# jayHuggie/PathTracer_CUDA_Interactive

Measured on AMD Instinct MI355X. Metric: Msamples/sec (rays x spp x bounces = intersect() calls per second), scenes/cbox/cbox.xml 640x480 spp=64, higher is better.
Workload: dtype f32

## Files before the change

pathtracer_cuda_interactive_amd/csrc/pt_api.hip:

```cpp
#include <cmath>
#include <cstdio>
#include <cstdlib>
#include <cstring>
#include <initializer_list>
#include <iterator>
#include <limits>
#include <mutex>
#include <type_traits>

#include "pt_scene.h"
#include "pt_transform.h"
#include "pt_denoise.h"
#include "pt_gradient.h"
#include "pt_temporal.h"
#include "pt_kernels.h"
#include "pt_kernel_q.h"
#include "pt_query.h"

using namespace ptk;

static thread_local std::string g_err;
int pt_fail(int code, const std::string& msg) { g_err = msg; return code; }
static int fail(int code, const std::string& msg) { return pt_fail(code, msg); }

// ... 249 lines not shown
    if (c.sched.inner >= 1000 && c.which != 1) return {};
    static_assert(std::size(kV2Schedules) == 9, "the index list below enumerates kV2Schedules");
    int si = -1;
    for (int k = 0; k < (int)std::size(kV2Schedules); k++)
        if (kV2Schedules[k].thresh == c.sched.thresh && kV2Schedules[k].inner == c.sched.inner && kV2Schedules[k].minw == c.sched.minw) si = k;
    return among<0, 1, 2, 3, 4, 5, 6, 7, 8>(si, [&](auto SI) { return among<0, 1, 2, 3>(c.res, [&](auto R) {
           return among<false, true>(c.nee, [&](auto N) { return among<false, true>(c.list, [&](auto LI) {
           static constexpr V2Schedule s = kV2Schedules[PT_CONST(SI)];
           if constexpr (!v2_compiled(PT_CONST(R), false, s, 0, PT_CONST(N), PT_CONST(LI))) return TraceEntry{};
           else return among<0, 1, 2>(c.spec, [&](auto SP) { return among<false, true>(c.prune, [&](auto P) {
           return among<false, true>(c.stats, [&](auto S) {
               if constexpr (v2_compiled(PT_CONST(R), PT_CONST(P), s, PT_CONST(SP), PT_CONST(N), PT_CONST(LI)))
                   return v2k<PT_CONST(R), PT_CONST(P), PT_CONST(S), s.thresh, s.inner, s.minw, PT_CONST(SP), PT_CONST(N), PT_CONST(LI)>();
               else return TraceEntry{}; }); }); }); }); }); }); });
}
#undef PT_CONST

void launch_trace(const pt_scene* S, const TraceChoice& c, const TraceEntry& e, int grid, hipStream_t stream, const RenderDev& rd,
                  const LdsPlan& lp, const QParams& qp, float4* samples) {
    void* const fn = const_cast<void*>(e.fn);
    if (c.family == 3)
        hipLaunchKernelGGL(reinterpret_cast<TraceFnQ>(fn), dim3(grid), dim3(c.block_threads), lp.total, stream, S->dev, rd, lp, qp,
                           samples, S->work_counter(), S->counters());
    else if (c.sweep)
        hipLaunchKernelGGL(reinterpret_cast<SweepFn>(fn), dim3(grid), dim3(c.block_threads), lp.total, stream, S->dev, rd, lp,
                           samples, S->work_counter(), S->counters(), SweepLayoutDev{S->sweep_tab.p, S->sweep.count, 0u});
    else
        hipLaunchKernelGGL(reinterpret_cast<TraceFn>(fn), dim3(grid), dim3(c.block_threads), lp.total, stream, S->dev, rd, lp,
                           samples, S->work_counter(), S->counters());
}

int read_slot_sums(const pt_scene* S, unsigned long long* out) {
    std::vector<unsigned long long> raw(kTimelineBase);
    HIP_TRY(hipMemcpy(raw.data(), S->counters(), raw.size() * sizeof(unsigned long long), hipMemcpyDeviceToHost));
    std::fill(out, out + kSlotStride, 0ull);
    for (int s = 0; s < kCounterSlots; s++)
        for (int k = 0; k < kSlotStride; k++) out[k] += raw[(size_t)s * kSlotStride + k];
    return PT_OK;
}

int launch_grid(int num_cus, int blocks_per_cu, uint64_t work_items, int block_threads = kBlock) {
    const uint64_t blocks_needed = (work_items + (uint64_t)block_threads - 1) / (uint64_t)block_threads;
    return (int)std::max<uint64_t>(1, std::min<uint64_t>((uint64_t)num_cus * (uint64_t)blocks_per_cu, blocks_needed));
}

struct RowSel {
    int begin, step, count;
};

int select_rows(const pt_render_params* p, RowSel* out) {
// ... 1190 lines not shown
    else if (k == "top_cache") S->opt_top_cache = value;
    else if (k == "fast_tree") S->opt_fast_tree = value;
    else if (k == "lds_budget_kb") S->opt_lds_budget_kb = value;
    else if (k == "chunk") S->opt_chunk = value;
    else if (k == "item_order") S->opt_item_order = value;
    else if (k == "specialize") S->opt_specialize = value;
    else if (k == "timing_frames") {
        if (value < 0 || value > 4096) return fail(PT_ERR_INVALID_ARG, "timing_frames must be 0 .. 4096");
        S->opt_timing_frames = value;
    }
    else if (k == "kernel") { if (value < 1 || value > 3) return fail(PT_ERR_INVALID_ARG, "kernel must be 1, 2 or 3"); S->opt_kernel = value; }
    else if (k == "frames_in_flight") {
        if (value < 1 || value > kMaxFramesInFlight) return fail(PT_ERR_INVALID_ARG, "frames_in_flight must be 1 .. " + std::to_string(kMaxFramesInFlight));
        S->opt_frames_in_flight = value;
    }
    else if (k == "q_target") S->opt_q_target = value;
    else if (k == "q_swap") S->opt_q_swap = value;
    else if (k == "q_low") S->opt_q_low = value;
    else if (k == "v2_thresh") S->opt_v2_thresh = value;
    else if (k == "v2_inner") S->opt_v2_inner = value;
    else if (k == "v2_minw") S->opt_v2_minw = value;
    else if (k == "reg_stack") { if (value != 0 && value != 1) return fail(PT_ERR_INVALID_ARG, "reg_stack must be 0 or 1"); S->opt_reg_stack = value; }
    else if (k == "leaf_sweep") { if (value != 0 && value != 1) return fail(PT_ERR_INVALID_ARG, "leaf_sweep must be 0 or 1"); S->opt_leaf_sweep = value; }
    else if (k == "query_refill") { if (value < 0 || value > 64) return fail(PT_ERR_INVALID_ARG, "query_refill must be 0 (automatic) .. 64"); S->opt_query_refill = value; }
    else if (k == "query_guides") { if (value < 0 || value > 2) return fail(PT_ERR_INVALID_ARG, "query_guides must be 0 (automatic), 1 or 2"); S->opt_query_guides = value; }
    else if (k == "query_blocks") { if (value < 0 || value > 4096) return fail(PT_ERR_INVALID_ARG, "query_blocks must be 0 (automatic) .. 4096"); S->opt_query_blocks = value; }
    else if (k == "tree_cost") { if (value != 0 && value != 1) return fail(PT_ERR_INVALID_ARG, "tree_cost must be 0 or 1"); S->opt_tree_cost = value; }
    else if (k == "rebuild_at_permille") {
        if (value != 0 && value < 1001) return fail(PT_ERR_INVALID_ARG, "rebuild_at_permille must be 0 (never) or at least 1001");
        S->opt_rebuild_at = value;
    }
    else return fail(PT_ERR_INVALID_ARG, "unknown option " + k);
    return PT_OK;
}

int pt_scene_get_info(pt_scene* S, const char* key, int64_t* value) {
    if (!S || !key || !value) return fail(PT_ERR_INVALID_ARG, "null argument");
    const std::string k(key);
    TraceChoice next;
    (void)choose_trace(S, k == "vgprs_pruned" ? PT_TRAVERSAL_PRUNED : PT_TRAVERSAL_EXACT, false, false, &next);
    DeviceGuard guard;
    unsigned long long c[kSlotStride];
    if (k == "grid") *value = S->info_grid;
    else if (k == "lds_bytes") *value = S->info_lds_bytes;
    else if (k == "lds_scene") *value = S->info_lds_scene;
    else if (k == "residency") *value = next.res;
// ... 29 lines not shown
    else if (k == "transforms") *value = S->transforms;
    else if (k == "rebuilds") *value = S->rebuilds;
    else if (k == "rebuilds_auto") *value = S->rebuilds_auto;
    else if (k == "rebuild_adopted") *value = S->rebuild_adopted;
    else if (k == "rebuild_cost_permille") *value = S->rebuild_cost_permille;
    else if (k == "tree_cost0_bits" || k == "tree_cost1_bits") {
        const int t = k[9] - '0';
        const double c = (S->cost_on() && (t == 0 || S->have_fast)) ? S->cost_now[t] : 0.0;
        *value = c > 0.0 ? __builtin_bit_cast(int64_t, c) : 0;
    }
    else if (k == "tree_cost0_permille" || k == "tree_cost1_permille") {
        const int t = k[9] - '0';
        *value = (S->cost_on() && (t == 0 || S->have_fast)) ? cost_permille(S, t) : 1000;
    }
    else if (k == "refit_shape0" || k == "refit_shape1") {
        const ptf::Plan& pl = S->refit_plan[k[11] - '0'];
        *value = !pl.built ? 0 : pl.whole_tree ? 1 : pl.narrow_top < pl.levels - 1 ? 2 : 3;
    }
    else if (k == "kernel") *value = S->info_kernel;
    else if (k == "trace_variant") *value = S->info_trace_variant;
    else if (k == "path_bank") *value = S->info_path_bank;
    else if (k == "leaf_sweep") *value = S->info_leaf_sweep;
    else if (k == "sweep_boxes") *value = S->sweep_groups;
    else if (k == "reg_stack") *value = S->info_reg_stack;
    else if (k == "block_threads") *value = S->info_kernel == 3 ? kQBlock : kBlock;
    else if (k == "frames_in_flight") *value = S->opt_frames_in_flight;
    else if (k == "query_chunk") *value = ptq::kQueryChunk;
    else if (k == "query_guides") *value = S->info_query_guides;
    else if (k == "query_grid") *value = S->info_query_grid;
    else if (k.rfind("qdiag", 0) == 0 && k.size() >= 6 && k.size() <= 7 && k.find_first_not_of("0123456789", 5) == std::string::npos &&
             std::stoi(k.substr(5)) < 11) {
        int rc = synced_slot_sums(S, guard, c);
        if (rc) return rc;
        *value = (int64_t)c[4 + std::stoi(k.substr(5))];
    }
    else if (k.rfind("diag", 0) == 0 && k.size() >= 5 && k.size() <= 7 && k.find_first_not_of("0123456789", 4) == std::string::npos &&
             std::stoi(k.substr(4)) < 8 + kNumCounters - kTimelineBase) {
        unsigned long long v = 0;
        const int idx = std::stoi(k.substr(4));
        if (idx < 8) {
            int rc = synced_slot_sums(S, guard, c);
            if (rc) return rc;
            v = c[4 + idx];
        } else {
            if (int grc = guard.enter(S->device)) return grc;
            HIP_TRY(hipStreamSynchronize(S->last_stream));
// ... 113 lines not shown
```

pathtracer_cuda_interactive_amd/csrc/pt_kernels.h:

```cpp
#pragma once

#include <hip/hip_runtime.h>

#include <type_traits>

#include "pt_layout.h"
#include "pt_leaf_sweep.h"
#include "pt_math.h"
#include "pt_path_bank.h"
#include "pt_path_index.h"
#include "pt_sweep_layout.h"
#include "pt_temporal.h"
#include "pt_trace.h"

namespace ptk {

using namespace ptl;


#ifndef PT_BLOCK
#define PT_BLOCK 256
#endif
constexpr int kBlock = PT_BLOCK;
constexpr uint32_t kMaxChunk = 256;

__device__ __forceinline__ uint32_t lane_rank(unsigned long long mask) {
    return __builtin_amdgcn_mbcnt_hi((uint32_t)(mask >> 32), __builtin_amdgcn_mbcnt_lo((uint32_t)mask, 0u));
}

__device__ __forceinline__ unsigned long long wave_sum(unsigned long long v) {
    for (int off = 32; off > 0; off >>= 1) v += __shfl_down(v, off, 64);
    return v;
}

// ... 247 lines not shown
    constexpr bool REG = false;
#include "pt_trace_v2_body.h"
}

template <int RES, bool PRUNE, bool STATS, int MINW>
__global__ __launch_bounds__(kBlock, (kBlock > 256 ? 1 : MINW)) void trace_kernel_v2_reg(SceneDev scn, RenderDev rp, LdsPlan lp,
                                                              float4* __restrict__ samples,
                                                              uint32_t* __restrict__ work_counter,
                                                              unsigned long long* __restrict__ counters) {
    constexpr int THRESH = 40, INNER = 162, SPEC = 2;
    constexpr bool NEE = false, LIST = false, REG = true;
#include "pt_trace_v2_body.h"
}

#ifndef PT_SWEEP_LEAF_STEPS
#define PT_SWEEP_LEAF_STEPS 4
#endif
#ifndef PT_SWEEP_THRESH
#define PT_SWEEP_THRESH 48
#endif
struct SweepLayoutDev {
    const unsigned char* tab;
    uint32_t groups;
    uint32_t pad;
};
struct SweepKernelArgs {
    SceneDev scn; RenderDev rp; LdsPlan lp; float4* samples; uint32_t* work_counter; unsigned long long* counters; SweepLayoutDev sweep;
};
static_assert(offsetof(SweepKernelArgs, rp) == offsetof(TraceKernelArgs, rp), "reload_render_args reads rp at TraceKernelArgs' offset");

__device__ __forceinline__ ptd::SceneView make_sweep_view(const SceneDev& scn, const LdsPlan& lp, const SweepLayoutDev& sweep,
                                                          unsigned char* smem) {
    const uint32_t slots_off = sweep_slots_off(sweep.groups);
    stage_to_lds(smem + lp.nodes_off, sweep.tab, slots_off);
    const DPrim* gslots = reinterpret_cast<const DPrim*>(sweep.tab + slots_off);
    DPrim* lslots = reinterpret_cast<DPrim*>(smem + lp.nodes_off + slots_off);
    for (uint32_t i = threadIdx.x; i < (uint32_t)scn.num_prims; i += blockDim.x) {
        const float4 a = ptd::ld4(gslots + i, 0), b = ptd::ld4(gslots + i, 1), c = ptd::ld4(gslots + i, 2);
        DPrim g;
        g.v[0] = a.x; g.v[1] = a.y; g.v[2] = a.z; g.v[3] = a.w; g.v[4] = b.x; g.v[5] = b.y; g.v[6] = b.z; g.v[7] = b.w; g.v[8] = c.x;
        g.info = __builtin_bit_cast(int32_t, c.y); g.light = __builtin_bit_cast(int32_t, c.z); g.pad = __builtin_bit_cast(int32_t, c.w);
        const DPrim r = sweep_stage_record(g);
        float4* d = reinterpret_cast<float4*>(lslots + i);
        d[0] = make_float4(r.v[0], r.v[1], r.v[2], r.v[3]);
        d[1] = make_float4(r.v[4], r.v[5], r.v[6], r.v[7]);
        d[2] = make_float4(r.v[8], c.y, c.z, c.w);
    }
    stage_to_lds(smem + lp.prims_off, scn.prims, (uint32_t)scn.num_prims * sizeof(DPrim));
    stage_to_lds(smem + lp.normals_off, scn.normals, (uint32_t)scn.num_prims * sizeof(DNormals));
    stage_to_lds(smem + lp.mats_off, scn.materials, (uint32_t)scn.num_materials * sizeof(DMaterial));
    stage_to_lds(smem + lp.emis_off, scn.emission, (uint32_t)scn.num_emission * sizeof(DEmission));
    __syncthreads();
    ptd::SceneView sv;
    sv.top_nodes = nullptr;
    sv.top_count = 0;
    sv.nodes = reinterpret_cast<const DNode*>(smem + lp.nodes_off);
    sv.prims = reinterpret_cast<const DPrim*>(smem + lp.prims_off);
    sv.normals = reinterpret_cast<const DNormals*>(smem + lp.normals_off);
    sv.materials = reinterpret_cast<const DMaterial*>(smem + lp.mats_off);
    sv.emission = reinterpret_cast<const DEmission*>(smem + lp.emis_off);
    sv.node_stride = kLdsNodeStride;
    sv.oct_stride = sweep_box_pitch(sweep.groups);
    sv.lights = scn.lights;
    sv.num_emission = scn.num_emission;
    sv.root_ref = scn.root_ref;
    sv.fixed_order = scn.fixed_order;
    sv.ref_nodes = scn.ref_nodes; sv.ref_path = scn.ref_path; sv.ref_anc = scn.ref_anc; sv.ref_levels = scn.ref_levels;
    sv.bg = ptm::mk(scn.bg[0], scn.bg[1], scn.bg[2]);
    return sv;
}

template <int MINW>
__global__ __launch_bounds__(kBlock, (kBlock > 256 ? 1 : MINW)) void trace_kernel_v2_sweep(SceneDev scn, RenderDev rp, LdsPlan lp,
                                                                float4* __restrict__ samples,
                                                                uint32_t* __restrict__ work_counter,
                                                                unsigned long long* __restrict__ counters,
                                                                SweepLayoutDev sweep) {
    constexpr int N_LEAF = PT_SWEEP_LEAF_STEPS;
#include "pt_trace_sweep_body.h"
}

__global__ __launch_bounds__(256) void resolve_kernel(const float4* __restrict__ samples, float* __restrict__ accum,
                                                      float* __restrict__ fb, uint32_t npix, int spp_pass,
                                                      int mode, int first, float scale) {
    const uint32_t pix = blockIdx.x * blockDim.x + threadIdx.x;
    if (pix >= npix) return;
    ptm::V3 sum = ptm::mk(0, 0, 0);
    if (mode != 2 && !first) sum = ptm::mk(accum[3 * (size_t)pix], accum[3 * (size_t)pix + 1], accum[3 * (size_t)pix + 2]);
    for (int s = 0; s < spp_pass; s++) {
        const float4 v = samples[(size_t)s * npix + pix];
        sum = sum + ptm::mk(v.x, v.y, v.z);
    }
// ... 304 lines not shown
```

pathtracer_cuda_interactive_amd/csrc/pt_scene.h:

```cpp
#pragma once
#include <hip/hip_runtime.h>

#include <algorithm>
#include <chrono>
#include <cstdint>
#include <string>
#include <utility>
#include <vector>

#include "../../include/pt_api.h"
#include "pt_internal.h"
#include "pt_layout.h"
#include "pt_leaf_sweep.h"
#include "pt_scene_refit.h"

#define HIP_TRY(expr)                                                                              \
    do {                                                                                           \
        hipError_t e_ = (expr);                                                                    \
        if (e_ != hipSuccess)                                                                      \
            return pt_fail(e_ == hipErrorNoDevice ? PT_ERR_NO_DEVICE : PT_ERR_DEVICE,              \
                           std::string(#expr) + ": " + hipGetErrorString(e_));                     \
    } while (0)

#define ENTER_DEVICE(S) DeviceGuard guard; if (int grc_ = guard.enter((S)->device)) return grc_

namespace ptkc {
constexpr int kBlock = 256, kCounterStride = 32, kQueryRing = 64, kLdsNodeStride = 64;
}

using namespace ptl;

template <class T>
struct DevBuf {
    T* p = nullptr;
    size_t n = 0;
    DevBuf() = default;
// ... 153 lines not shown
            if (f.in_ev) (void)hipEventDestroy(f.in_ev);
            f.stream = nullptr; f.free_ev = nullptr; f.in_ev = nullptr; f.used = false;
        }
    }
    hipStream_t last_stream = nullptr;
    bool have_timing = false;
    int64_t opt_blocks_per_cu = 0;
    int64_t opt_scratch_bytes = 0;
    int64_t opt_force_global = 0;
    int64_t opt_stats = 0;
    int64_t opt_specialize = 1;
    int64_t opt_octants = 1;
    int64_t opt_top_cache = 1;
    int64_t opt_fast_tree = 1;
    int64_t opt_chunk = 0;
    int64_t opt_lds_budget_kb = 0;
    int64_t opt_item_order = 1;
    int64_t opt_xcd_regions = 0;
    int64_t opt_kernel = 2;
    int64_t opt_q_target = 0, opt_q_swap = 0, opt_q_low = 0;
    int64_t opt_v2_thresh = 0, opt_v2_inner = 0, opt_v2_minw = 0;
    int64_t opt_reg_stack = 1;
    int64_t opt_leaf_sweep = 1;
    SweepTable sweep{};
    int sweep_groups = 0;
    DevBuf<unsigned char> sweep_tab;
    int64_t create_us[7] = {0, 0, 0, 0, 0, 0, 0}, sweep_on_device = 0;
    int64_t info_grid = 0, info_lds_bytes = 0, info_lds_scene = 0, info_passes = 0, info_occupancy = 0, info_blocks_per_cu = 0, info_debug_reruns = 0, fast_cost_permille = 0, info_kernel = 0, info_trace_variant = 0, info_path_bank = 0, info_reg_stack = 0, info_leaf_sweep = 0;
    struct PassEvents { hipEvent_t t0, t1, r0, r1; };
    struct FrameRec { std::vector<PassEvents> ev; size_t passes = 0; };
    std::vector<FrameRec> frames;
    uint64_t frame_seq = 0;
    int64_t opt_timing_frames = 1;
    const FrameRec* last_frame() const { return frame_seq && !frames.empty() ? &frames[(frame_seq - 1) % frames.size()] : nullptr; }
    void drop_events() {
        for (auto& f : frames)
            for (auto& pe : f.ev) { (void)hipEventDestroy(pe.t0); (void)hipEventDestroy(pe.t1); (void)hipEventDestroy(pe.r0); (void)hipEventDestroy(pe.r1); }
        frames.clear();
        frame_seq = 0;
    }
    const void* cfg_fn = nullptr;
    uint32_t cfg_lds = 0;
    int cfg_occ = 0;
    ~pt_scene() {
        drop_query();
        for (auto& T : tree) { T.nodes.release(); T.nodes_oct.release(); }
        drop_slots(); drop_events();
        prims.release(); normals.release(); materials.release(); emission.release(); lights.release();
        for (auto& pl : refit_plan) ptf::plan_release(&pl);
// ... 31 lines not shown
```

pathtracer_cuda_interactive_amd/csrc/pt_scene_life.hip:

```cpp
#include <cmath>
#include <cstdlib>
#include <cstring>
#include <exception>
#include <limits>
#include <queue>

#include "pt_scene.h"
#include "pt_tree_sweep.h"
#include "pt_sweep_build.h"
#include "pt_scene_prep.h"
#include "pt_tree_cost.h"
#include "pt_scene_transform.h"
#include "pt_transform.h"
#include "pt_sweep_layout.h"

namespace {
using namespace ptkc;

constexpr uint32_t kOctNodeLimit = 24 * 1024;
constexpr int kMaxStack = 64;
constexpr int kMinInternalTree = 16;
constexpr int kDeviceSweepMin = 4096;
#ifndef PT_TOP_NODES
#define PT_TOP_NODES 512
#endif
constexpr uint32_t kTopNodes = PT_TOP_NODES;
constexpr uint32_t kMaxLdsBudget = 160 * 1024;

bool prepared_on_device(int N) {
    const char* v = std::getenv("PT_SWEEP_BUILD");
    return N >= kDeviceSweepMin && !(v && std::string(v) == "host");
}

struct TreeHost {
    std::vector<DNode> nodes;
    int32_t root_ref = 0;
    int depth = 1;
// ... 268 lines not shown
    std::vector<pt_bvh_node> fnodes;
    int32_t froot = 0, fdepth = 0;
    bool ok = true, fnested = true;
    try {
        pts::build_sweep_tree(boxes_host, N, fnodes, &froot, &fdepth);
    } catch (const std::exception&) {
        ok = false;
    }
    built(try_device);
    c.ok = ok && convert_tree(fnodes.data(), (int)fnodes.size(), froot, N, c.host, nullptr, &fnested, true) == PT_OK && fnested;
    return c;
}

void drop_internal_tree(pt_scene* S, const char* why) {
    S->have_fast = S->fast_is_callers_topology = false;
    S->no_fast_why = why;
    S->tree[1].nodes.release(); S->tree[1].nodes_oct.release(); S->tree[1].have_oct = false;
    S->ref_path.release(); S->ref_anc.release();
}

int64_t probe_permille(const unsigned long long v[2]) { return v[0] ? (int64_t)((1000ull * v[1] + v[0] / 2) / v[0]) : 1000; }
bool probe_wins(const unsigned long long v[2]) { return v[1] * 100ull < v[0] * 90ull; }

int make_sweep_tables(const TreeHost& fast, const DPrim* prims, int N, SweepTable& sweep, int& sweep_groups, DevBuf<unsigned char>& sweep_tab) {
    sweep = SweepTable{};
    sweep_groups = 0;
    SweepGroup groups[kSweepMaxPrims];
    const int n = build_sweep_groups(fast.nodes.data(), (int)fast.nodes.size(), N, kLdsNodeStride, groups);
    if (n > 0) {
        sweep_groups = n;
        std::vector<unsigned char> tab(n <= kSweepMaxBoxes ? sweep_layout_bytes((uint32_t)n, (uint32_t)N) : 0);
        if (n <= kSweepMaxBoxes && build_sweep_layout(groups, n, fast.nodes.data(), (int)fast.nodes.size(), kLdsNodeStride, prims, N, tab.data())) {
            if (int rc = sweep_tab.ensure(tab.size())) return rc;
            HIP_TRY(hipMemcpy(sweep_tab.p, tab.data(), tab.size(), hipMemcpyHostToDevice));
            sweep.count = (uint32_t)n;
            std::copy(groups, groups + n, sweep.g);
        }
    }
    return PT_OK;
}

int check_desc(const pt_scene_desc* d) {
    if (!d) return pt_fail(PT_ERR_INVALID_ARG, "null scene description");
    if (d->num_shapes <= 0 || !d->shapes) return pt_fail(PT_ERR_BAD_SCENE, "scene has no shapes");
    if (d->num_nodes != 2 * d->num_shapes - 1 || !d->nodes)
        return pt_fail(PT_ERR_BAD_SCENE, "BVH must have 2*num_shapes-1 nodes (bvh.cu:16-54)");
    if (d->root < 0 || d->root >= d->num_nodes) return pt_fail(PT_ERR_BAD_SCENE, "BVH root out of range");
    if (d->num_materials <= 0 || !d->materials) return pt_fail(PT_ERR_BAD_SCENE, "scene has no materials");
    if (d->num_meshes < 0 || (d->num_meshes > 0 && !d->meshes)) return pt_fail(PT_ERR_BAD_SCENE, "bad mesh array");
    if (d->num_lights < 0 || (d->num_lights > 0 && !d->lights)) return pt_fail(PT_ERR_BAD_SCENE, "bad light array");
    if (int rc = check_materials(d)) return rc;
    return check_meshes(d, d->num_materials);
}

struct CreateState {
    bool on_device = false, nested = true;
    std::vector<DPrim> prims; std::vector<DNormals> normals;
// ... 139 lines not shown
    S->diffuse_only = all_diffuse(d);
    S->create_us[1] = clock.lap();
    if ((rc = callers_tree(d, S, c))) return rc;
    S->create_us[2] = clock.lap();
    if (N < kMinInternalTree) {
        S->no_fast_why = "fewer than 16 shapes";
    } else if (!c.nested) {
        S->no_fast_why = "the caller's boxes do not nest";
    } else {
        c.cand = internal_tree(c.boxes_dev.p, c.on_device ? nullptr : c.boxes_host.data(), N,
                               [&](bool again) { if (!again) S->create_us[3] = clock.lap(); });
        if (!c.cand.ok) S->no_fast_why = "the internal tree could not be built";
    }
    S->sweep_on_device = c.cand.on_device ? 1 : 0;
    c.boxes_dev.release();
    std::vector<float>().swap(c.boxes_host);
    S->create_us[4] = clock.lap();
    if ((rc = upload_scene(d, S, c))) return rc;
    if ((rc = probe_and_decide(d, S, c.ref_inner))) return rc;
    S->create_us[5] = clock.lap();
    if ((rc = tie_tables(d, S, c))) return rc;
    S->sweep = SweepTable{}; S->sweep_groups = 0;
    if (S->have_fast && !c.cand.on_device && !S->fast_is_callers_topology && N <= kSweepMaxPrims &&
        (rc = make_sweep_tables(c.cand.host, c.prims.data(), N, S->sweep, S->sweep_groups, S->sweep_tab)))
        return rc;
    HIP_TRY(hipDeviceSynchronize());
    S->create_us[6] = clock.lap(); S->create_us[0] = clock.total();
    select_tree(S, 0);
    S->scene_bytes = (uint32_t)std::min<size_t>(
        c.ref_inner * sizeof(DNode) + (size_t)N * (sizeof(DPrim) + sizeof(DNormals)) + (size_t)d->num_materials * sizeof(DMaterial) +
            (size_t)std::max(d->num_lights, 1) * sizeof(DEmission) + 64, 0xffffffffu);
    return PT_OK;
}

int ensure_staging(pt_scene* S) {
    const size_t N = (size_t)S->dev.num_prims;
    int rc;
    if ((rc = S->st_prims.ensure(N)) || (rc = S->prev_prims.ensure(N)) || (rc = S->st_normals.ensure(N))) return rc;
    return S->st_status.ensure(1);
}

int ensure_cost(pt_scene* S) {
    int rc;
    const size_t need = std::max(ptc::partials_needed(S->tree[0].num_nodes), ptc::partials_needed(S->tree[1].num_nodes));
    if ((rc = S->cost_partials.ensure(need)) || (rc = S->cost_dev.ensure(4))) return rc;
    if (!S->cost_host) HIP_TRY(hipHostMalloc(reinterpret_cast<void**>(&S->cost_host), 4 * sizeof(double), hipHostMallocDefault));
    return PT_OK;
// ... 41 lines not shown
    HIP_TRY(hipMemsetAsync(S->st_status.p, 0, sizeof(unsigned int), nullptr));
    unsigned int bad = 0;
    if (!whole || n_trees == 0) {
        if ((rc = S->st_boxes.ensure((size_t)N * 6)) || (rc = ptf::leaf_boxes(S->st_prims.p, N, S->st_boxes.p, S->st_status.p))) return rc;
        HIP_TRY(hipMemcpy(&bad, S->st_status.p, sizeof bad, hipMemcpyDeviceToHost));
    }
    for (int t = 0; t < n_trees && !bad; t++) {
        pt_scene::Tree& T = S->tree[t];
        if ((rc = ptf::refit_tree(S->refit_plan[t], T.nodes.p, T.have_oct ? T.nodes_oct.p : nullptr, T.num_nodes, S->st_prims.p,
                                  whole ? nullptr : S->st_boxes.p, N, S->st_status.p)))
            return rc;
    }
    if (whole && n_trees) HIP_TRY(hipMemcpy(&bad, S->st_status.p, sizeof bad, hipMemcpyDeviceToHost));
    if (bad) return pt_fail(PT_ERR_UNSUPPORTED, std::string(who) + ": a new coordinate, radius or leaf box is not finite");
    for (int t = 0; costs && t < n_trees; t++) S->cost_pending_now[t] = enqueue_cost(S, S->tree[t], 2 + t) == PT_OK;
    S->prev_prims.swap(S->st_prims);
    S->prims.swap(S->prev_prims);
    S->have_prev = true;
    S->normals.swap(S->st_normals);
    S->dev.prims = S->prims.p; S->dev.normals = S->normals.p;
    S->tri_only = tri_only;
    S->sweep_groups = 0; S->sweep.count = 0;
    S->sweep_tab.release();
    *us_refit = clock.lap();
    return PT_OK;
}

int rebuild_scene(pt_scene* S) {
    if (!S->have_fast)
        return pt_fail(PT_ERR_UNSUPPORTED, std::string("pt_scene_rebuild: the handle holds no tie tables, pt_scene_create kept no internal tree: ") +
                                               (S->no_fast_why[0] ? S->no_fast_why : "none was built"));
    const int N = S->dev.num_prims;
    const pt_scene::Tree& T0 = S->tree[0];
    StageClock clock;
    int64_t us[4] = {0, 0, 0, 0};
    int rc;
    DevBuf<float> boxes_dev;
    if ((rc = boxes_dev.ensure((size_t)N * 6)) || (rc = ptf::tree_leaf_boxes(T0.nodes.p, T0.num_nodes, N, boxes_dev.p))) return rc;
    InternalTree cand = internal_tree(boxes_dev.p, nullptr, N, [&](bool again) { if (again) clock.rewind(); us[1] = clock.lap(); });
    if (cand.copy_error != hipSuccess)
        return pt_fail(cand.copy_error == hipErrorNoDevice ? PT_ERR_NO_DEVICE : PT_ERR_DEVICE, std::string("hipMemcpy(leaf_boxes.data(), boxes_dev.p, leaf_boxes.size() * sizeof(float), hipMemcpyDeviceToHost): ") + hipGetErrorString(cand.copy_error));
    if (!cand.ok)
        return pt_fail(PT_ERR_UNSUPPORTED, "pt_scene_rebuild: no internal tree could be built of the leaf boxes (not finite, or they no longer nest)");
    if (!cand.on_device && (rc = upload_tree(cand.tree, cand.host))) return rc;
    boxes_dev.release();
    SceneDev d0 = S->dev, d1 = S->dev;
    tree_view(S, d0, 0, false);
    tree_view(S, d1, cand.tree, 1, false);
    for (SceneDev* dv : {&d0, &d1}) { dv->ref_path = nullptr; dv->ref_anc = nullptr; dv->ref_levels = 0; dv->redo_stack = nullptr; }
    unsigned long long v[2] = {0, 0};
    if ((rc = probe_trees(d0, d1, v))) return rc;
    const bool adopt = probe_wins(v);
    us[2] = clock.lap();
    ptf::Plan plan;
    SweepTable sweep{}; int sweep_groups = 0; DevBuf<unsigned char> sweep_tab;
    double cost = 0.0;
    if (adopt) {
        if (S->refit_plan[1].built && (rc = ptf::plan_build(cand.tree.nodes.p, cand.tree.num_nodes, N, &plan))) return rc;
        struct PlanGuard { ptf::Plan* p; ~PlanGuard() { if (p) ptf::plan_release(p); } } plan_guard{&plan};
        if (!cand.on_device && N <= kSweepMaxPrims) {
            std::vector<DPrim> prims((size_t)N);
            HIP_TRY(hipMemcpy(prims.data(), S->prims.p, prims.size() * sizeof(DPrim), hipMemcpyDeviceToHost));
            if ((rc = make_sweep_tables(cand.host, prims.data(), N, sweep, sweep_groups, sweep_tab))) return rc;
        }
        if (S->cost_on()) {
            if ((rc = ensure_cost(S)) || (rc = enqueue_cost(S, cand.tree, 3))) return rc;
            HIP_TRY(hipStreamSynchronize(nullptr));
            cost = S->cost_host[3];
        }
        std::swap(S->tree[1], cand.tree);
        S->have_fast = true; S->fast_is_callers_topology = false;
        S->fast_cost_permille = probe_permille(v);
        S->sweep_on_device = cand.on_device ? 1 : 0;
        std::swap(S->refit_plan[1], plan);
        plan_guard.p = &plan;
        S->sweep = sweep; S->sweep_groups = sweep_groups;
        S->sweep_tab.swap(sweep_tab);
        S->cfg_fn = S->q_cfg_fn = nullptr;
        if (S->cost_on()) { S->cost_ref[1] = S->cost_now[1] = cost; S->cost_have_ref[1] = true; }
    } else if (S->cost_have_ref[1] && S->cost_now[1] > 0.0) {
        S->cost_ref[1] = S->cost_now[1];
    }
    us[3] = clock.lap();
    us[0] = clock.total();
    select_tree(S, 0);
    S->rebuilds++; S->rebuild_adopted = adopt ? 1 : 0; S->rebuild_cost_permille = probe_permille(v);
    std::copy(us, us + 4, S->rebuild_us);
    return PT_OK;
}

void rebuild_by_policy(pt_scene* S) {
    if (S->opt_rebuild_at <= 0 || !S->have_fast || !S->cost_pending_now[1]) return;
    if (hipStreamSynchronize(nullptr) != hipSuccess) return;
    collect_costs(S);
    if (cost_permille(S, 1) < S->opt_rebuild_at) return;
    if (rebuild_scene(S) == PT_OK) S->rebuilds_auto++;
}

int update_scene(pt_scene* S, const pt_scene_desc* d, int flags) {
    const bool geometry = (flags & PT_UPDATE_GEOMETRY) != 0, shading = (flags & PT_UPDATE_SHADING) != 0;
// ... 216 lines not shown
```

pathtracer_cuda_interactive_amd/csrc/pt_trace_sweep_body.h:

```cpp
    extern __shared__ __attribute__((aligned(16))) unsigned char smem[];
    constexpr int THRESH = PT_SWEEP_THRESH;
    typedef const __attribute__((address_space(3))) unsigned char* LdsBytes;
    typedef float f2v __attribute__((ext_vector_type(2)));
    typedef const __attribute__((address_space(3))) f2v* LdsF2;
    const uint32_t n_groups = sweep.groups;
    const uint32_t box_pitch = sweep_box_pitch(n_groups);
    const ptd::SceneView sv = make_sweep_view(scn, lp, sweep, smem);
    const ptd::lds_f4v* slots = (const ptd::lds_f4v*)(smem + lp.nodes_off + sweep_slots_off(n_groups));

    const int lane = threadIdx.x & 63;
    const int wave = threadIdx.x >> 6;

    WorkFeed feed;
    feed_init(feed, rp);
    PathBank bank;
    bank_init(bank);
    float bank_dx = 0.0f, bank_dy = 0.0f, bank_dz = 0.0f;
    uint32_t bank_lo = 0, bank_hi = 0;
    uint32_t bank_w = 0, bank_inc_lo = 0, bank_inc_hi = 0;
    bool alive = false;
    ptd::Ray ray;
    ray.org = ptm::mk(0, 0, 0); ray.dir = ptm::mk(0, 0, 1); ray.tnear = 0; ray.tfar = 0;
    ptd::Trav tv;
    tv.inv = ptm::mk(1, 1, 1);
    tv.best.t = 0; tv.best.u = 0; tv.best.v = 0; tv.best.prim = -1;
    tv.cur = 0; tv.stack_state = 0; tv.node_off = 0; tv.redo = false;
    uint32_t hits = 0;
    uint32_t pend = 0;
    ptm::V3 L = ptm::mk(0, 0, 0), T = ptm::mk(1, 1, 1);
// ... 70 lines not shown
                    L = ptm::mk(0, 0, 0);
                    T = ptm::mk(1, 1, 1);
                    depth = 0;
                    alive = true;
                }
                n_paths += k;
                want = __ballot(idle && !alive);
            }
            n_segs += (uint32_t)__popcll(__ballot(idle && alive));
            if (idle && alive) {
                const ptm::V3 inv = ptm::mk(ptm::rcp_exact(ray.dir.x), ptm::rcp_exact(ray.dir.y), ptm::rcp_exact(ray.dir.z));
                tv.best.t = FLT_MAX; tv.best.u = 0.0f; tv.best.v = 0.0f; tv.best.prim = -1;
                tv.redo = !(__builtin_isfinite(inv.x) && __builtin_isfinite(inv.y) && __builtin_isfinite(inv.z));
                if (!tv.redo) {
                    const uint32_t oct = (inv.x < 0.0f ? 1u : 0u) | (inv.y < 0.0f ? 2u : 0u) | (inv.z < 0.0f ? 4u : 0u);
                    LdsF2 bx = (LdsF2)((LdsBytes)smem + lp.nodes_off + oct * box_pitch);
                    const ptm::V3 o = ray.org;
                    auto box_sides = [&](const f2v p0, const f2v p1, const f2v p2, float& tf, float& tn0) {
                        const float tn = ptm::fmax2(ptm::fmax2((p0.x - o.x) * inv.x, (p0.y - o.y) * inv.y), (p1.x - o.z) * inv.z);
                        tf = ptm::fmin2(ptm::fmin2((p1.y - o.x) * inv.x, (p2.x - o.y) * inv.y), (p2.y - o.z) * inv.z);
                        tn0 = ptm::fmax2(0.0f, tn);
                    };
                    uint32_t h = 0;
#pragma clang loop vectorize(disable) interleave(disable) unroll(disable)
                    for (uint32_t k = n_groups >> 1; k != 0; k--) {
                        const f2v a0 = bx[0], a1 = bx[1], a2 = bx[2], b0 = bx[3], b1 = bx[4], b2 = bx[5];
                        bx += 6;
                        float tfa, tna, tfb, tnb;
                        box_sides(a0, a1, a2, tfa, tna);
                        box_sides(b0, b1, b2, tfb, tnb);
                        unsigned long long mb;
                        asm("v_cmp_ge_f32_e32 vcc, %2, %3\n\t"
                            "v_cmp_ge_f32_e64 %1, %4, %5\n\t"
                            "s_nop 0\n\t"
                            "v_addc_co_u32_e32 %0, vcc, %0, %0, vcc\n\t"
                            "v_addc_co_u32_e64 %0, vcc, %0, %0, %1"
                            : "+v"(h), "=&s"(mb) : "v"(tfa), "v"(tna), "v"(tfb), "v"(tnb) : "vcc");
                    }
                    if (n_groups & 1u) {
                        float tf, tn0;
                        box_sides(bx[0], bx[1], bx[2], tf, tn0);
                        asm("v_cmp_ge_f32_e32 vcc, %1, %2\n\ts_nop 1\n\tv_addc_co_u32_e32 %0, vcc, %0, %0, vcc" : "+v"(h) : "v"(tf), "v"(tn0) : "vcc");
                    }
                    hits = sweep_hits_align(h, n_groups);
                }
            }
        }
#pragma unroll
        for (int k = 0; k < N_LEAF; k++) {
            if ((hits | pend) != 0u) {
                uint32_t slot = pend;
                if (pend == 0u) {
                    slot = sweep_first_group(hits);
                    hits = sweep_clear_group(hits, slot);
                }
                pend = ptd::leaf_test_slot(sv, slots, ray, tv, slot);
            }
        }
    }
    flush_counters<false>(counters, lane, lane == 0 ? n_paths : 0u, lane == 0 ? n_segs : 0u, st);
```

Measured before the change: 44240.

## Pair sweep boxes sharing an axis slab to cut LDS loads and slab math

Builds an alternative sweep table where leaf-group boxes with identical min/max planes on one axis are paired and stored compactly (10 floats per pair, with flat slabs computing one plane). The ray sweep loop now runs specialized per-axis loops over these shared/flat pairs before the general pairs, reducing LDS reads and subtract-multiply work per box test. This adds six extra loop prologues per ray, an extra device table, and a greedy host-side pairing pass at build time; it is enabled by default via a new option.

```diff
diff --git a/pathtracer_cuda_interactive_amd/csrc/pt_api.hip b/pathtracer_cuda_interactive_amd/csrc/pt_api.hip
--- a/pathtracer_cuda_interactive_amd/csrc/pt_api.hip
+++ b/pathtracer_cuda_interactive_amd/csrc/pt_api.hip
@@ -295,10 +295,13 @@
     if (c.family == 3)
         hipLaunchKernelGGL(reinterpret_cast<TraceFnQ>(fn), dim3(grid), dim3(c.block_threads), lp.total, stream, S->dev, rd, lp, qp,
                            samples, S->work_counter(), S->counters());
-    else if (c.sweep)
+    else if (c.sweep) {
+        const bool pairs = S->opt_sweep_pairs && S->sweep_tab_pairs.p;
+        const SweepPairClasses cls = pairs ? S->sweep_classes : sweep_pairs_none(S->sweep.count);
         hipLaunchKernelGGL(reinterpret_cast<SweepFn>(fn), dim3(grid), dim3(c.block_threads), lp.total, stream, S->dev, rd, lp,
-                           samples, S->work_counter(), S->counters(), SweepLayoutDev{S->sweep_tab.p, S->sweep.count, 0u});
-    else
+                           samples, S->work_counter(), S->counters(),
+                           SweepLayoutDev{pairs ? S->sweep_tab_pairs.p : S->sweep_tab.p, S->sweep.count, sweep_pairs_pitch(cls), cls});
+    } else
         hipLaunchKernelGGL(reinterpret_cast<TraceFn>(fn), dim3(grid), dim3(c.block_threads), lp.total, stream, S->dev, rd, lp,
                            samples, S->work_counter(), S->counters());
 }
@@ -1535,6 +1538,7 @@
     else if (k == "v2_minw") S->opt_v2_minw = value;
     else if (k == "reg_stack") { if (value != 0 && value != 1) return fail(PT_ERR_INVALID_ARG, "reg_stack must be 0 or 1"); S->opt_reg_stack = value; }
     else if (k == "leaf_sweep") { if (value != 0 && value != 1) return fail(PT_ERR_INVALID_ARG, "leaf_sweep must be 0 or 1"); S->opt_leaf_sweep = value; }
+    else if (k == "sweep_pairs") { if (value != 0 && value != 1) return fail(PT_ERR_INVALID_ARG, "sweep_pairs must be 0 or 1"); S->opt_sweep_pairs = value; }
     else if (k == "query_refill") { if (value < 0 || value > 64) return fail(PT_ERR_INVALID_ARG, "query_refill must be 0 (automatic) .. 64"); S->opt_query_refill = value; }
     else if (k == "query_guides") { if (value < 0 || value > 2) return fail(PT_ERR_INVALID_ARG, "query_guides must be 0 (automatic), 1 or 2"); S->opt_query_guides = value; }
     else if (k == "query_blocks") { if (value < 0 || value > 4096) return fail(PT_ERR_INVALID_ARG, "query_blocks must be 0 (automatic) .. 4096"); S->opt_query_blocks = value; }
@@ -1610,6 +1614,15 @@
     else if (k == "path_bank") *value = S->info_path_bank;
     else if (k == "leaf_sweep") *value = S->info_leaf_sweep;
     else if (k == "sweep_boxes") *value = S->sweep_groups;
+    else if (k.rfind("sweep_share_pairs", 0) == 0 || k.rfind("sweep_flat_pairs", 0) == 0 || k == "sweep_general_pairs") {
+        const SweepPairClasses c = !S->sweep.count ? SweepPairClasses{} : S->opt_sweep_pairs && S->sweep_tab_pairs.p ? S->sweep_classes : sweep_pairs_none(S->sweep.count);
+        const bool flat = k[6] == 'f';
+        const std::string axis = k.substr(flat ? 16 : 17);
+        if (k == "sweep_general_pairs") *value = c.general;
+        else if (axis.empty()) *value = flat ? sweep_pairs_flat(c) : sweep_pairs_shared(c);
+        else if (axis == "_x" || axis == "_y" || axis == "_z") *value = (flat ? c.flat : c.share)[axis[1] - 'x'];
+        else return fail(PT_ERR_INVALID_ARG, "unknown info key " + k);
+    }
     else if (k == "reg_stack") *value = S->info_reg_stack;
     else if (k == "block_threads") *value = S->info_kernel == 3 ? kQBlock : kBlock;
     else if (k == "frames_in_flight") *value = S->opt_frames_in_flight;
diff --git a/pathtracer_cuda_interactive_amd/csrc/pt_kernels.h b/pathtracer_cuda_interactive_amd/csrc/pt_kernels.h
--- a/pathtracer_cuda_interactive_amd/csrc/pt_kernels.h
+++ b/pathtracer_cuda_interactive_amd/csrc/pt_kernels.h
@@ -10,6 +10,7 @@
 #include "pt_path_bank.h"
 #include "pt_path_index.h"
 #include "pt_sweep_layout.h"
+#include "pt_sweep_pairs.h"
 #include "pt_temporal.h"
 #include "pt_trace.h"
 
@@ -303,7 +304,8 @@
 struct SweepLayoutDev {
     const unsigned char* tab;
     uint32_t groups;
-    uint32_t pad;
+    uint32_t box_pitch;
+    SweepPairClasses classes;
 };
 struct SweepKernelArgs {
     SceneDev scn; RenderDev rp; LdsPlan lp; float4* samples; uint32_t* work_counter; unsigned long long* counters; SweepLayoutDev sweep;
@@ -341,7 +343,7 @@
     sv.materials = reinterpret_cast<const DMaterial*>(smem + lp.mats_off);
     sv.emission = reinterpret_cast<const DEmission*>(smem + lp.emis_off);
     sv.node_stride = kLdsNodeStride;
-    sv.oct_stride = sweep_box_pitch(sweep.groups);
+    sv.oct_stride = sweep.box_pitch;
     sv.lights = scn.lights;
     sv.num_emission = scn.num_emission;
     sv.root_ref = scn.root_ref;
@@ -349,6 +351,36 @@
     sv.ref_nodes = scn.ref_nodes; sv.ref_path = scn.ref_path; sv.ref_anc = scn.ref_anc; sv.ref_levels = scn.ref_levels;
     sv.bg = ptm::mk(scn.bg[0], scn.bg[1], scn.bg[2]);
     return sv;
+}
+
+typedef float SweepF2 __attribute__((ext_vector_type(2)));
+typedef const __attribute__((address_space(3))) SweepF2* SweepLdsF2;
+template <int A> __device__ __forceinline__ float sweep_axis(const ptm::V3& v) { return A == 0 ? v.x : A == 1 ? v.y : v.z; }
+template <int AX, bool FLAT>
+__device__ __forceinline__ SweepLdsF2 sweep_shared_pairs(SweepLdsF2 bx, uint32_t count, const ptm::V3& o, const ptm::V3& inv, uint32_t& h) {
+    constexpr int B = AX == 0 ? 1 : 0, C = AX == 2 ? 1 : 2;
+    const float oa = sweep_axis<AX>(o), ia = sweep_axis<AX>(inv), ob = sweep_axis<B>(o), ib = sweep_axis<B>(inv), oc = sweep_axis<C>(o), ic = sweep_axis<C>(inv);
+#pragma clang loop vectorize(disable) interleave(disable) unroll(disable)
+    for (uint32_t k = count; k != 0; k--) {
+        const SweepF2 s = bx[0], an = bx[1], af = bx[2], bn = bx[3], bf = bx[4];
+        bx += 5;
+        float na[3], fa[3], nb[3], fb[3];
+        na[AX] = (s.x - oa) * ia;
+        fa[AX] = FLAT ? na[AX] : (s.y - oa) * ia;
+        nb[AX] = na[AX]; fb[AX] = fa[AX];
+        na[B] = (an.x - ob) * ib; na[C] = (an.y - oc) * ic; fa[B] = (af.x - ob) * ib; fa[C] = (af.y - oc) * ic;
+        nb[B] = (bn.x - ob) * ib; nb[C] = (bn.y - oc) * ic; fb[B] = (bf.x - ob) * ib; fb[C] = (bf.y - oc) * ic;
+        const float tfa = ptm::fmin2(ptm::fmin2(fa[0], fa[1]), fa[2]), tna = ptm::fmax2(0.0f, ptm::fmax2(ptm::fmax2(na[0], na[1]), na[2]));
+        const float tfb = ptm::fmin2(ptm::fmin2(fb[0], fb[1]), fb[2]), tnb = ptm::fmax2(0.0f, ptm::fmax2(ptm::fmax2(nb[0], nb[1]), nb[2]));
+        unsigned long long mb;
+        asm("v_cmp_ge_f32_e32 vcc, %2, %3\n\t"
+            "v_cmp_ge_f32_e64 %1, %4, %5\n\t"
+            "s_nop 0\n\t"
+            "v_addc_co_u32_e32 %0, vcc, %0, %0, vcc\n\t"
+            "v_addc_co_u32_e64 %0, vcc, %0, %0, %1"
+            : "+v"(h), "=&s"(mb) : "v"(tfa), "v"(tna), "v"(tfb), "v"(tnb) : "vcc");
+    }
+    return bx;
 }
 
 template <int MINW>
diff --git a/pathtracer_cuda_interactive_amd/csrc/pt_scene.h b/pathtracer_cuda_interactive_amd/csrc/pt_scene.h
--- a/pathtracer_cuda_interactive_amd/csrc/pt_scene.h
+++ b/pathtracer_cuda_interactive_amd/csrc/pt_scene.h
@@ -12,6 +12,7 @@
 #include "pt_internal.h"
 #include "pt_layout.h"
 #include "pt_leaf_sweep.h"
+#include "pt_sweep_pairs.h"
 #include "pt_scene_refit.h"
 
 #define HIP_TRY(expr)                                                                              \
@@ -211,9 +212,12 @@
     int64_t opt_v2_thresh = 0, opt_v2_inner = 0, opt_v2_minw = 0;
     int64_t opt_reg_stack = 1;
     int64_t opt_leaf_sweep = 1;
+    int64_t opt_sweep_pairs = 1;
     SweepTable sweep{};
     int sweep_groups = 0;
     DevBuf<unsigned char> sweep_tab;
+    DevBuf<unsigned char> sweep_tab_pairs;
+    SweepPairClasses sweep_classes{};
     int64_t create_us[7] = {0, 0, 0, 0, 0, 0, 0}, sweep_on_device = 0;
     int64_t info_grid = 0, info_lds_bytes = 0, info_lds_scene = 0, info_passes = 0, info_occupancy = 0, info_blocks_per_cu = 0, info_debug_reruns = 0, fast_cost_permille = 0, info_kernel = 0, info_trace_variant = 0, info_path_bank = 0, info_reg_stack = 0, info_leaf_sweep = 0;
     struct PassEvents { hipEvent_t t0, t1, r0, r1; };
diff --git a/pathtracer_cuda_interactive_amd/csrc/pt_scene_life.hip b/pathtracer_cuda_interactive_amd/csrc/pt_scene_life.hip
--- a/pathtracer_cuda_interactive_amd/csrc/pt_scene_life.hip
+++ b/pathtracer_cuda_interactive_amd/csrc/pt_scene_life.hip
@@ -13,6 +13,7 @@
 #include "pt_scene_transform.h"
 #include "pt_transform.h"
 #include "pt_sweep_layout.h"
+#include "pt_sweep_pairs.h"
 
 namespace {
 using namespace ptkc;
@@ -327,17 +328,31 @@
 int64_t probe_permille(const unsigned long long v[2]) { return v[0] ? (int64_t)((1000ull * v[1] + v[0] / 2) / v[0]) : 1000; }
 bool probe_wins(const unsigned long long v[2]) { return v[1] * 100ull < v[0] * 90ull; }
 
-int make_sweep_tables(const TreeHost& fast, const DPrim* prims, int N, SweepTable& sweep, int& sweep_groups, DevBuf<unsigned char>& sweep_tab) {
+int make_sweep_tables(const TreeHost& fast, const DPrim* prims, int N, SweepTable& sweep, int& sweep_groups, DevBuf<unsigned char>& sweep_tab,
+                      DevBuf<unsigned char>& sweep_tab_pairs, SweepPairClasses& classes) {
     sweep = SweepTable{};
     sweep_groups = 0;
+    classes = SweepPairClasses{};
     SweepGroup groups[kSweepMaxPrims];
     const int n = build_sweep_groups(fast.nodes.data(), (int)fast.nodes.size(), N, kLdsNodeStride, groups);
     if (n > 0) {
         sweep_groups = n;
         std::vector<unsigned char> tab(n <= kSweepMaxBoxes ? sweep_layout_bytes((uint32_t)n, (uint32_t)N) : 0);
-        if (n <= kSweepMaxBoxes && build_sweep_layout(groups, n, fast.nodes.data(), (int)fast.nodes.size(), kLdsNodeStride, prims, N, tab.data())) {
+        SweepGroup paired[kSweepMaxBoxes];
+        int perm[kSweepMaxBoxes];
+        SweepPairClasses cls{};
+        std::vector<unsigned char> tab_pairs(tab.size());
+        const DNode* nodes = fast.nodes.data();
+        const int num_nodes = (int)fast.nodes.size();
+        if (n <= kSweepMaxBoxes && build_sweep_layout(groups, n, nodes, num_nodes, kLdsNodeStride, prims, N, tab.data()) &&
+            build_sweep_pairs(groups, n, nodes, num_nodes, kLdsNodeStride, paired, perm, &cls) &&
+            build_sweep_layout(paired, n, nodes, num_nodes, kLdsNodeStride, prims, N, tab_pairs.data()) &&
+            build_sweep_pair_tables(paired, n, cls, nodes, num_nodes, kLdsNodeStride, tab_pairs.data())) {
             if (int rc = sweep_tab.ensure(tab.size())) return rc;
+            if (int rc = sweep_tab_pairs.ensure(tab_pairs.size())) return rc;
             HIP_TRY(hipMemcpy(sweep_tab.p, tab.data(), tab.size(), hipMemcpyHostToDevice));
+            HIP_TRY(hipMemcpy(sweep_tab_pairs.p, tab_pairs.data(), tab_pairs.size(), hipMemcpyHostToDevice));
+            classes = cls;
             sweep.count = (uint32_t)n;
             std::copy(groups, groups + n, sweep.g);
         }
@@ -523,7 +538,7 @@
     if ((rc = tie_tables(d, S, c))) return rc;
     S->sweep = SweepTable{}; S->sweep_groups = 0;
     if (S->have_fast && !c.cand.on_device && !S->fast_is_callers_topology && N <= kSweepMaxPrims &&
-        (rc = make_sweep_tables(c.cand.host, c.prims.data(), N, S->sweep, S->sweep_groups, S->sweep_tab)))
+        (rc = make_sweep_tables(c.cand.host, c.prims.data(), N, S->sweep, S->sweep_groups, S->sweep_tab, S->sweep_tab_pairs, S->sweep_classes)))
         return rc;
     HIP_TRY(hipDeviceSynchronize());
     S->create_us[6] = clock.lap(); S->create_us[0] = clock.total();
@@ -611,6 +626,7 @@
     S->tri_only = tri_only;
     S->sweep_groups = 0; S->sweep.count = 0;
     S->sweep_tab.release();
+    S->sweep_tab_pairs.release(); S->sweep_classes = SweepPairClasses{};
     *us_refit = clock.lap();
     return PT_OK;
 }
@@ -642,7 +658,7 @@
     const bool adopt = probe_wins(v);
     us[2] = clock.lap();
     ptf::Plan plan;
-    SweepTable sweep{}; int sweep_groups = 0; DevBuf<unsigned char> sweep_tab;
+    SweepTable sweep{}; int sweep_groups = 0; DevBuf<unsigned char> sweep_tab, sweep_tab_pairs; SweepPairClasses sweep_classes{};
     double cost = 0.0;
     if (adopt) {
         if (S->refit_plan[1].built && (rc = ptf::plan_build(cand.tree.nodes.p, cand.tree.num_nodes, N, &plan))) return rc;
@@ -650,7 +666,7 @@
         if (!cand.on_device && N <= kSweepMaxPrims) {
             std::vector<DPrim> prims((size_t)N);
             HIP_TRY(hipMemcpy(prims.data(), S->prims.p, prims.size() * sizeof(DPrim), hipMemcpyDeviceToHost));
-            if ((rc = make_sweep_tables(cand.host, prims.data(), N, sweep, sweep_groups, sweep_tab))) return rc;
+            if ((rc = make_sweep_tables(cand.host, prims.data(), N, sweep, sweep_groups, sweep_tab, sweep_tab_pairs, sweep_classes))) return rc;
         }
         if (S->cost_on()) {
             if ((rc = ensure_cost(S)) || (rc = enqueue_cost(S, cand.tree, 3))) return rc;
@@ -665,6 +681,7 @@
         plan_guard.p = &plan;
         S->sweep = sweep; S->sweep_groups = sweep_groups;
         S->sweep_tab.swap(sweep_tab);
+        S->sweep_tab_pairs.swap(sweep_tab_pairs); S->sweep_classes = sweep_classes;
         S->cfg_fn = S->q_cfg_fn = nullptr;
         if (S->cost_on()) { S->cost_ref[1] = S->cost_now[1] = cost; S->cost_have_ref[1] = true; }
     } else if (S->cost_have_ref[1] && S->cost_now[1] > 0.0) {
diff --git a/pathtracer_cuda_interactive_amd/csrc/pt_sweep_pairs.h b/pathtracer_cuda_interactive_amd/csrc/pt_sweep_pairs.h
--- /dev/null
+++ b/pathtracer_cuda_interactive_amd/csrc/pt_sweep_pairs.h
@@ -0,0 +1,138 @@
+#pragma once
+#include <stdint.h>
+#include <string.h>
+
+#include "pt_sweep_layout.h"
+
+namespace ptl {
+
+constexpr uint32_t kSweepPairFloats = 12, kSweepSharedPairFloats = 10, kSweepSingleFloats = 6;
+constexpr int kSweepSavingFlat = 6, kSweepSavingShare = 4;
+
+struct SweepPairClasses {
+    uint8_t flat[3];
+    uint8_t share[3];
+    uint8_t general;
+    uint8_t single;
+};
+static_assert(sizeof(SweepPairClasses) == 8, "SweepPairClasses travels as two scalar words");
+
+PT_SWEEP_HD uint32_t sweep_pairs_shared(const SweepPairClasses& c) { return (uint32_t)c.share[0] + c.share[1] + c.share[2]; }
+PT_SWEEP_HD uint32_t sweep_pairs_flat(const SweepPairClasses& c) { return (uint32_t)c.flat[0] + c.flat[1] + c.flat[2]; }
+PT_SWEEP_HD uint32_t sweep_pairs_groups(const SweepPairClasses& c) {
+    return 2u * (sweep_pairs_shared(c) + sweep_pairs_flat(c) + c.general) + c.single;
+}
+PT_SWEEP_HD SweepPairClasses sweep_pairs_none(uint32_t groups) {
+    SweepPairClasses c{};
+    c.general = (uint8_t)(groups >> 1);
+    c.single = (uint8_t)(groups & 1u);
+    return c;
+}
+PT_SWEEP_HD uint32_t sweep_pairs_pitch(const SweepPairClasses& c) {
+    const uint32_t bytes = 4u * (kSweepSharedPairFloats * (sweep_pairs_shared(c) + sweep_pairs_flat(c)) + kSweepPairFloats * c.general +
+                                 kSweepSingleFloats * c.single);
+    return bytes + (((bytes / 8u) & 1u) ? 0u : 8u);
+}
+
+inline const float* sweep_group_box(const SweepGroup& g, const DNode* nodes, int num_nodes, uint32_t node_stride) {
+    const uint32_t node = g.box_off / node_stride, rest = g.box_off % node_stride;
+    if (node >= (uint32_t)num_nodes || (rest != 0 && rest != kSweepBoxBytes)) return nullptr;
+    return rest ? nodes[node].rmin : nodes[node].lmin;
+}
+
+inline int sweep_pair_saving(const float* a, const float* b, int* axis) {
+    int best = 0;
+    *axis = -1;
+    for (int x = 0; x < 3; x++) {
+        if (memcmp(a + x, b + x, 4) != 0 || memcmp(a + 3 + x, b + 3 + x, 4) != 0) continue;
+        const int s = memcmp(a + x, a + 3 + x, 4) == 0 ? kSweepSavingFlat : kSweepSavingShare;
+        if (s > best) { best = s; *axis = x; }
+    }
+    return best;
+}
+
+inline bool build_sweep_pairs(const SweepGroup* groups, int count, const DNode* nodes, int num_nodes, uint32_t node_stride,
+                              SweepGroup* out, int* perm, SweepPairClasses* classes) {
+    if (count < 1 || count > kSweepMaxBoxes) return false;
+    const float* box[kSweepMaxBoxes];
+    for (int k = 0; k < count; k++)
+        if (!(box[k] = sweep_group_box(groups[k], nodes, num_nodes, node_stride))) return false;
+    bool used[kSweepMaxBoxes] = {};
+    int pair_of[6][kSweepMaxBoxes];
+    int n_of[6] = {0, 0, 0, 0, 0, 0};
+    for (;;) {
+        int best = 0, bi = -1, bj = -1, ba = -1;
+        for (int i = 0; i < count; i++) {
+            if (used[i]) continue;
+            for (int j = i + 1; j < count; j++) {
+                if (used[j]) continue;
+                int axis;
+                const int s = sweep_pair_saving(box[i], box[j], &axis);
+                if (s > best) { best = s; bi = i; bj = j; ba = axis; }
+            }
+        }
+        if (best == 0) break;
+        const int cls = (best == kSweepSavingFlat ? 0 : 3) + ba;
+        pair_of[cls][n_of[cls]++] = bi;
+        pair_of[cls][n_of[cls]++] = bj;
+        used[bi] = used[bj] = true;
+    }
+    int n = 0;
+    SweepPairClasses c{};
+    for (int cls = 0; cls < 6; cls++) {
+        for (int k = 0; k < n_of[cls]; k++) perm[n++] = pair_of[cls][k];
+        (cls < 3 ? c.flat[cls] : c.share[cls - 3]) = (uint8_t)(n_of[cls] / 2);
+    }
+    const int paired = n;
+    for (int k = 0; k < count; k++)
+        if (!used[k]) perm[n++] = k;
+    c.general = (uint8_t)((count - paired) / 2);
+    c.single = (uint8_t)((count - paired) & 1);
+    for (int k = 0; k < count; k++) out[k] = groups[perm[k]];
+    *classes = c;
+    return true;
+}
+
+inline bool build_sweep_pair_tables(const SweepGroup* groups, int count, const SweepPairClasses& classes, const DNode* nodes,
+                                    int num_nodes, uint32_t node_stride, unsigned char* out) {
+    if (count < 1 || count > kSweepMaxBoxes || sweep_pairs_groups(classes) != (uint32_t)count || classes.single > 1) return false;
+    const uint32_t pitch = sweep_pairs_pitch(classes);
+    if (8u * pitch > sweep_slots_off((uint32_t)count)) return false;
+    memset(out, 0, sweep_slots_off((uint32_t)count));
+    for (uint32_t o = 0; o < 8; o++) {
+        float* w = reinterpret_cast<float*>(out + o * pitch);
+        int k = 0;
+        auto planes = [&](int g, float* nf) {
+            const float* box = sweep_group_box(groups[g], nodes, num_nodes, node_stride);
+            if (!box) return false;
+            for (int a = 0; a < 3; a++) {
+                const bool neg = (o >> a) & 1u;
+                nf[a] = box[neg ? 3 + a : a];
+                nf[3 + a] = box[neg ? a : 3 + a];
+            }
+            return true;
+        };
+        for (int cls = 0; cls < 6; cls++) {
+            const int ax = cls % 3, b = ax == 0 ? 1 : 0, c = ax == 2 ? 1 : 2;
+            const bool flat = cls < 3;
+            for (int p = 0; p < (flat ? classes.flat[ax] : classes.share[ax]); p++, k += 2) {
+                float A[6], B[6];
+                if (!planes(k, A) || !planes(k + 1, B)) return false;
+                if (memcmp(&A[ax], &B[ax], 4) != 0 || memcmp(&A[3 + ax], &B[3 + ax], 4) != 0) return false;
+                if (flat && memcmp(&A[ax], &A[3 + ax], 4) != 0) return false;
+                const float rec[kSweepSharedPairFloats] = {A[ax], flat ? 0.0f : A[3 + ax], A[b], A[c], A[3 + b], A[3 + c], B[b], B[c], B[3 + b], B[3 + c]};
+                memcpy(w, rec, sizeof(rec));
+                w += kSweepSharedPairFloats;
+            }
+        }
+        for (int p = 0; p < 2 * classes.general + classes.single; p++, k++) {
+            float A[6];
+            if (!planes(k, A)) return false;
+            memcpy(w, A, sizeof(A));
+            w += kSweepSingleFloats;
+        }
+    }
+    return true;
+}
+
+}
diff --git a/pathtracer_cuda_interactive_amd/csrc/pt_trace_sweep_body.h b/pathtracer_cuda_interactive_amd/csrc/pt_trace_sweep_body.h
--- a/pathtracer_cuda_interactive_amd/csrc/pt_trace_sweep_body.h
+++ b/pathtracer_cuda_interactive_amd/csrc/pt_trace_sweep_body.h
@@ -4,7 +4,8 @@
     typedef float f2v __attribute__((ext_vector_type(2)));
     typedef const __attribute__((address_space(3))) f2v* LdsF2;
     const uint32_t n_groups = sweep.groups;
-    const uint32_t box_pitch = sweep_box_pitch(n_groups);
+    const uint32_t box_pitch = sweep.box_pitch;
+    const uint64_t cls_bits = __builtin_bit_cast(uint64_t, sweep.classes);
     const ptd::SceneView sv = make_sweep_view(scn, lp, sweep, smem);
     const ptd::lds_f4v* slots = (const ptd::lds_f4v*)(smem + lp.nodes_off + sweep_slots_off(n_groups));
 
@@ -121,8 +122,20 @@
                         tn0 = ptm::fmax2(0.0f, tn);
                     };
                     uint32_t h = 0;
+                    uint32_t cls_lo = (uint32_t)cls_bits, cls_hi = (uint32_t)(cls_bits >> 32);
+                    asm volatile("" : "+s"(cls_lo), "+s"(cls_hi));
+                    SweepPairClasses cls;
+                    cls.flat[0] = (uint8_t)cls_lo; cls.flat[1] = (uint8_t)(cls_lo >> 8); cls.flat[2] = (uint8_t)(cls_lo >> 16);
+                    cls.share[0] = (uint8_t)(cls_lo >> 24); cls.share[1] = (uint8_t)cls_hi; cls.share[2] = (uint8_t)(cls_hi >> 8);
+                    cls.general = (uint8_t)(cls_hi >> 16); cls.single = (uint8_t)(cls_hi >> 24);
+                    bx = sweep_shared_pairs<0, true>(bx, cls.flat[0], o, inv, h);
+                    bx = sweep_shared_pairs<1, true>(bx, cls.flat[1], o, inv, h);
+                    bx = sweep_shared_pairs<2, true>(bx, cls.flat[2], o, inv, h);
+                    bx = sweep_shared_pairs<0, false>(bx, cls.share[0], o, inv, h);
+                    bx = sweep_shared_pairs<1, false>(bx, cls.share[1], o, inv, h);
+                    bx = sweep_shared_pairs<2, false>(bx, cls.share[2], o, inv, h);
 #pragma clang loop vectorize(disable) interleave(disable) unroll(disable)
-                    for (uint32_t k = n_groups >> 1; k != 0; k--) {
+                    for (uint32_t k = cls.general; k != 0; k--) {
                         const f2v a0 = bx[0], a1 = bx[1], a2 = bx[2], b0 = bx[3], b1 = bx[4], b2 = bx[5];
                         bx += 6;
                         float tfa, tna, tfb, tnb;
@@ -136,7 +149,7 @@
                             "v_addc_co_u32_e64 %0, vcc, %0, %0, %1"
                             : "+v"(h), "=&s"(mb) : "v"(tfa), "v"(tna), "v"(tfb), "v"(tnb) : "vcc");
                     }
-                    if (n_groups & 1u) {
+                    if (cls.single) {
                         float tf, tn0;
                         box_sides(bx[0], bx[1], bx[2], tf, tn0);
                         asm("v_cmp_ge_f32_e32 vcc, %1, %2\n\ts_nop 1\n\tv_addc_co_u32_e32 %0, vcc, %0, %0, vcc" : "+v"(h) : "v"(tf), "v"(tn0) : "vcc");
```

After: 45260, median of 6. 1.02x the previous value.
